# chayanchatterjee/GW-Whisper

Hardware: AMD Instinct MI355X
Metric: 1s-strain segments/sec (encoder fwd) (higher is better)
Workload: dtype bf16; 1 GPU; whisper-tiny encoder fwd, batch 256 log-mel (80x3000) per GPU, 1500 tokens, random-init weights (BASELINE configs[1]); global_batch=256, parallelism=dp1, encoder=tiny, streams_per_gpu=1

## Files before the change

### gw_whisper_amd/csrc/mlp_fused.hip

```cpp
#include "common.h"

#include <stdlib.h>

#include <type_traits>

namespace gww {

namespace {
constexpr int MF_D = 384;
constexpr int MF_KT = MF_D / 64;
constexpr int MF_OT = MF_D / 32;
constexpr int MF_WAVES = 4, MF_THREADS = 256, MF_BM = 128;
#ifndef GWW_MF_EXP
#define GWW_MF_EXP 0
#endif
#ifndef GWW_MF_ABL
#define GWW_MF_ABL 0
#endif
#ifndef GWW_MF_OLDDMA
#define GWW_MF_OLDDMA 0
#endif
#ifndef GWW_MF_AHEAD
#define GWW_MF_AHEAD 3
#endif
#ifndef GWW_MF_SCHED
#define GWW_MF_SCHED 1
#endif
#ifndef GWW_MF_VACC
#define GWW_MF_VACC 1
#endif
#ifndef GWW_MF_NTSTORE
#define GWW_MF_NTSTORE 1
#endif
#ifndef GWW_MF_NTLOAD
#define GWW_MF_NTLOAD 1
#endif
#if GWW_MF_NTLOAD
#define MF_NT " nt"
#else
#define MF_NT ""
#endif
#ifndef GWW_MF_PADNOP
#define GWW_MF_PADNOP 0
#endif
#if GWW_MF_PADNOP
#define MF_PADNOP "s_nop 1\n\t"
#else
#define MF_PADNOP ""
#endif
#ifndef GWW_MF_XLDS
#define GWW_MF_XLDS 0
#endif
#ifndef GWW_MF_XSTNT
#define GWW_MF_XSTNT 0
#endif
#ifndef GWW_MF_XNT
#define GWW_MF_XNT 0
#endif
#if GWW_MF_XNT
#define MF_XNT MF_NT
#else
#define MF_XNT ""
#endif
#ifndef GWW_MF_DMAGAP
#define GWW_MF_DMAGAP 1
#endif
#ifndef GWW_MF_TAIL2
#define GWW_MF_TAIL2 0
#endif
#ifndef GWW_MF_NORM
#define GWW_MF_NORM 1
#endif
#ifndef GWW_MF_XACC
#define GWW_MF_XACC 1
#endif
constexpr int MF_AHEAD = GWW_MF_AHEAD;
constexpr int MF_NST_MAX = MF_AHEAD + 1;
constexpr int MF_TILE = 128 * 64 * 2;
constexpr int MF_GL = 16 / MF_WAVES;
constexpr int MF_FMAX = 1536;
constexpr int MF_SLICE_STRIDE = 144, MF_SLICE_BYTES = 32 * MF_SLICE_STRIDE;
constexpr int MF_OFF_CB = MF_NST_MAX * MF_TILE;
constexpr int MF_OFF_U = MF_OFF_CB + MF_FMAX * 4;
constexpr int MF_OFF_B2 = MF_OFF_U + MF_FMAX * 4;
constexpr int MF_OFF_BO = MF_OFF_B2 + MF_D * 4;
constexpr int MF_OFF_QCB = MF_OFF_BO + MF_D * 4;
constexpr int MF_OFF_SLICE = MF_OFF_QCB + MF_FMAX * 4;
constexpr int MF_LDS = MF_OFF_SLICE + 2 * MF_WAVES * MF_SLICE_BYTES;
static_assert(MF_LDS <= 160 * 1024, "LDS budget");

template <int N>
using MF_FL = std::integral_constant<int, N>;

__device__ __forceinline__ float mf_sum8(float v) {
  v += __builtin_bit_cast(float, __builtin_amdgcn_update_dpp(0, __builtin_bit_cast(int, v), 0xB1, 0xF, 0xF, true));
  v += __builtin_bit_cast(float, __builtin_amdgcn_update_dpp(0, __builtin_bit_cast(int, v), 0x4E, 0xF, 0xF, true));
  v += __builtin_bit_cast(float, __builtin_amdgcn_update_dpp(0, __builtin_bit_cast(int, v), 0x141, 0xF, 0xF, true));
  return v;
}

template <int N>
__device__ __forceinline__ void mf_wait_vmcnt() {
  asm volatile("s_waitcnt vmcnt(%0)" ::"n"(N) : "memory");
}

__device__ __forceinline__ float gelu_sig(float x) {
  const float s = fminf(x * x, 64.0f);
  float q = fmaf(s, 0.0010148164f, -0.1067791331f);
  q = fmaf(s, q, -2.3011178f);
#if GWW_MF_EXP & 32
  const float e = (x * q) * 0.37f;
  return x * ((1.0f + e) * 0.91f);
#else
  const float e = __builtin_amdgcn_exp2f(x * q);
  return x * __builtin_amdgcn_rcpf(1.0f + e);
#endif
}

#ifdef GWW_STAMP
__device__ unsigned long long g_stamp_mlp[24];
#define MSTAMP_DECL unsigned long long _t0 = __builtin_amdgcn_s_memtime(); unsigned long long _acc[20] = {0}; \
  const unsigned long long _tb = _t0, _rb = __builtin_amdgcn_s_memrealtime();
#define MSTAMP(i)                                                  \
  do {                                                             \
    if (GWW_STAMP >= 2 && (i) != 0 && (i) != 3 && (i) != 4 && (i) != 5 && !((i) >= 100)) break; \
    __builtin_amdgcn_sched_barrier(0);                             \
    const unsigned long long _t1 = __builtin_amdgcn_s_memtime();   \
    _acc[(i) >= 100 ? (i) - 100 : (i)] += _t1 - _t0;               \
    _t0 = _t1;                                                     \
    __builtin_amdgcn_sched_barrier(0);                             \
  } while (0)
#define TSTAMP(i) do { if (GWW_STAMP == 3) MSTAMP(100 + (i)); } while (0)
#define MSTAMP_FLUSH                                                                 \
  if (lane == 0) {                                                                   \
    for (int _q = 0; _q < 20; ++_q) atomicAdd(&g_stamp_mlp[_q], _acc[_q]);           \
    atomicAdd(&g_stamp_mlp[21], __builtin_amdgcn_s_memrealtime() - _rb);             \
    atomicAdd(&g_stamp_mlp[22], __builtin_amdgcn_s_memtime() - _tb);                 \
    atomicAdd(&g_stamp_mlp[23], 1ull);                                                \
  }
#else
#define MSTAMP_DECL
#define MSTAMP(i)
#define TSTAMP(i)
#define MSTAMP_FLUSH
#endif
}

__device__ __forceinline__ const float* mf_x0_row(const MfX0& z, const float* X, long g, bool x0, bool& tail, int& seg) {
  tail = false; seg = 0;
  if (!x0) return X + g * MF_D;
  const unsigned b = (unsigned)g / (unsigned)z.T, j = (unsigned)g - b * (unsigned)z.T;
  seg = (int)b;
  tail = (int)j >= z.Tt - 2 && (int)j <= z.T - 2;
  if (tail) return z.pos + (long)j * MF_D;
  return z.xs + ((long)b * z.Tt + ((int)j == z.T - 1 ? z.Tt - 1 : (int)j)) * MF_D;
}

struct MfNoX0 {};
template <int MODE, bool OP, bool X0 = false>
__global__ __launch_bounds__(MF_THREADS, 1) void k_mlp_fused(const float* X, const unsigned short* delta, float* x_out,
                                                            const float* __restrict__ ln_u,
                                                            const float* __restrict__ ln_cb,
                                                            const unsigned short* __restrict__ Wt,
                                                            const float* __restrict__ b2,
                                                            unsigned short* __restrict__ C, long M, int F,
                                                            int stagger_ticks, const float* __restrict__ q_u,
                                                            const float* __restrict__ q_cb,
                                                            unsigned short* __restrict__ q_out, int NQ,
                                                            float* x_next, const float* __restrict__ bo, int keep_x_new,
                                                            const std::conditional_t<X0, MfX0, MfNoX0> z) {
  __shared__ __attribute__((aligned(16))) unsigned char lds[MF_LDS];
  constexpr bool QKV = MODE == 1 || MODE == 2, LNQ = MODE == 2, FIN = MODE == 3;
  static_assert(!X0 || (GWW_MF_NORM && GWW_MF_XACC && (MODE == 2 || (MODE == 1 && OP))), "X0: layer 0's two launches; stages in the u table");
  constexpr bool XACC = GWW_MF_XACC && GWW_MF_NORM && GWW_MF_SCHED && OP && (MODE == 1 || MODE == 3);
  constexpr int MF_NST = MF_AHEAD + 1;
  float* lds_cb = reinterpret_cast<float*>(lds + MF_OFF_CB);
  float* lds_u = reinterpret_cast<float*>(lds + MF_OFF_U);
  float* lds_b2 = reinterpret_cast<float*>(lds + MF_OFF_B2);
  float* lds_bo = reinterpret_cast<float*>(lds + MF_OFF_BO);
  float* lds_qcb = reinterpret_cast<float*>(lds + MF_OFF_QCB);
  constexpr int OP_TILES = OP ? 3 * MF_KT : 0;
  typedef __attribute__((address_space(3))) void* lds_ptr;

  const int tid = threadIdx.x, lane = tid & 63, wave = tid >> 6;
  const int r = lane & 31, hh = lane >> 5;
  const long m_base = (long)blockIdx.x * MF_BM + wave * 32;
  unsigned char* slice = lds + MF_OFF_SLICE + wave * MF_SLICE_BYTES;
  unsigned char* const slice0 = slice;
  const int crow = lane >> 3, cchunk = lane & 7;

  const int wave_u = __builtin_amdgcn_readfirstlane(wave);
  const unsigned lane_off = (unsigned)lane * 16u;
  const unsigned lds_base = (unsigned)(unsigned long long)(lds_ptr)lds;
  auto issue_piece_c = [&](int tile, int stage, auto j_c) {
    constexpr int J = decltype(j_c)::value;
    const unsigned dst = lds_base + (unsigned)(stage * MF_TILE + MF_GL * wave_u * 1024);
    if (GWW_MF_EXP & 8) tile &= 7;
    const unsigned short* src = Wt + ((long)tile * (MF_TILE / 2) + MF_GL * wave_u * 512);
    const unsigned lo = lane_off;
    asm volatile("s_mov_b32 m0, %2\n\ts_nop 0\n\tglobal_load_lds_dwordx4 %0, %1 offset:%3"
                 :
                 : "v"(lo), "s"(src), "s"(dst), "n"(J * 1024)
                 : "memory");
  };
  auto issue_piece = [&](int tile, int stage, int j) {
#if GWW_MF_OLDDMA
    const unsigned dst = lds_base + (unsigned)(stage * MF_TILE + (MF_GL * wave_u + j) * 1024);
    const unsigned short* src = Wt + ((long)tile * (MF_TILE / 2) + (MF_GL * wave_u + j) * 512);
    unsigned keep;
    asm volatile("s_mov_b32 %0, m0\n\ts_mov_b32 m0, %3\n\ts_nop 0\n\tglobal_load_lds_dwordx4 %1, %2\n\ts_mov_b32 m0, %0"
                 : "=&s"(keep) : "v"(lane_off), "s"(src), "s"(dst) : "memory");
#else
    if (j == 0) issue_piece_c(tile, stage, std::integral_constant<int, 0>{});
    else if (j == 1) issue_piece_c(tile, stage, std::integral_constant<int, 1>{});
    else if (j == 2) issue_piece_c(tile, stage, std::integral_constant<int, 2>{});
    else issue_piece_c(tile, stage, std::integral_constant<int, 3>{});
#endif
  };
  auto issue = [&](int tile, int stage) {
#pragma unroll
    for (int j = 0; j < MF_GL; ++j) issue_piece(tile, stage, j);
  };

  MSTAMP_DECL
  auto stage_tables = [&]() {
    for (int i = tid; i < F; i += MF_THREADS) {
      lds_cb[i] = GWW_MF_SCHED ? ln_cb[i] * 0.125f : ln_cb[i];
      if (!GWW_MF_NORM) lds_u[i] = ln_u[i];
    }
    if (!GWW_MF_NORM && FIN) __syncthreads();
    if (!LNQ)
      for (int i = tid; i < MF_D; i += MF_THREADS) lds_b2[i] = XACC ? b2[i] + bo[i] : b2[i];
    if (OP)
      for (int i = tid; i < MF_D; i += MF_THREADS) lds_bo[i] = bo[i];
    if (FIN)
      for (int i = tid; i < MF_D; i += MF_THREADS) { lds_u[i] = q_u[i]; lds_u[MF_D + i] = q_cb[i]; }
    if (QKV && GWW_MF_NORM)
      for (int i = tid; i < NQ; i += MF_THREADS) lds_qcb[i] = q_cb[i];
  };
  if constexpr (!XACC) stage_tables();
  if (stagger_ticks > 0 && blockIdx.x < 256) {
    const unsigned long long t0 = __builtin_amdgcn_s_memrealtime();
    const unsigned long long wait = (unsigned long long)((blockIdx.x >> 3) & 15) * stagger_ticks;
    while (__builtin_amdgcn_s_memrealtime() - t0 < wait) __builtin_amdgcn_s_sleep(8);
  }

#pragma unroll
  for (int p = 0; p < MF_AHEAD; ++p) issue(p, p);
  const long xrow_l = m_base + r < M ? m_base + r : M - 1;
  const unsigned xoff = (unsigned)xrow_l * (unsigned)(MF_D * 4) + 16u * (unsigned)hh;
  f32x4 xp[XACC ? MF_OT : 1][4];
  bool x0 = false;
  int x0_seg0 = 0;
  f32x4* const lds_x0 = reinterpret_cast<f32x4*>(lds + MF_OFF_U);
  const float* x0_stage[2] = {nullptr, nullptr};
  f32x4 x0_sg[2];
  bool x0_tail = false;
  int x0_seg = 0;
  if constexpr (X0) {
    x0 = __builtin_amdgcn_readfirstlane(*z.flag) != 0;
    const unsigned g0 = (unsigned)blockIdx.x * (unsigned)MF_BM;
    x0_seg0 = (int)(g0 / (unsigned)z.T);
    const int seg_last = (int)((unsigned)(M - 1) / (unsigned)z.T);
#pragma unroll
    for (int k = 0; k < 2; ++k) {
      const int q = tid + 256 * k < 4 * (MF_D / 4) ? tid + 256 * k : tid;
      const int sg = q / (2 * (MF_D / 4)), wh = (q / (MF_D / 4)) & 1, c = q % (MF_D / 4);
      const long b = x0_seg0 + sg < seg_last ? x0_seg0 + sg : seg_last;
      x0_stage[k] = (wh ? z.tr + b * MF_D : z.xs + (b * z.Tt + (z.Tt - 2)) * MF_D) + 4 * c;
    }
  }
  auto x0_publish = [&](f32x4 (&sg)[2]) {
    lds_x0[tid] = sg[0];
    if (tid + 256 < 4 * (MF_D / 4)) lds_x0[tid + 256] = sg[1];
    asm volatile("s_waitcnt lgkmcnt(0)" ::: "memory");
    __builtin_amdgcn_s_barrier();
    asm volatile("" ::: "memory");
  };
  if constexpr (XACC && X0) {
    const float* xsrc = mf_x0_row(z, X, xrow_l, x0, x0_tail, x0_seg) + 4 * hh;
#pragma unroll
    for (int t = 0; t < MF_OT; ++t)
#pragma unroll
      for (int cc = 0; cc < 4; ++cc)
        asm volatile("global_load_dwordx4 %0, %1, off offset:%2" MF_XNT : "=a"(xp[t][cc]) : "v"(xsrc), "n"((32 * t + 8 * cc) * 4) : "memory");
#pragma unroll
    for (int k = 0; k < 2; ++k) asm volatile("global_load_dwordx4 %0, %1, off" : "=v"(x0_sg[k]) : "v"(x0_stage[k]) : "memory");
  } else if constexpr (XACC) {
#pragma unroll
    for (int t = 0; t < MF_OT; ++t)
#pragma unroll
      for (int cc = 0; cc < 4; ++cc)
        if (GWW_MF_ABL & 32) asm volatile("v_accvgpr_write_b32 %0, 0" : "=a"(xp[t][cc][0]));
        else asm volatile("global_load_dwordx4 %0, %1, %2 offset:%3" MF_XNT : "=a"(xp[t][cc]) : "v"(xoff), "s"(X), "n"((32 * t + 8 * cc) * 4) : "memory");
  }
  bf16x8 af[MF_KT * 4];
  float row_rstd, row_mean;
  long grow[4];
#pragma unroll
  for (int i = 0; i < 4; ++i) {
    const long g = m_base + 8 * i + crow;
    grow[i] = g < M ? g : M - 1;
  }
  if constexpr (XACC) {
    const unsigned coff = (unsigned)xrow_l * (unsigned)(MF_D * 2) + 64u * (unsigned)hh;
#pragma unroll
    for (int S = 0; S < MF_KT; ++S)
#pragma unroll
      for (int j = 0; j < 4; ++j)
        asm volatile("global_load_dwordx4 %0, %1, %2 offset:%3" : "=v"(af[4 * S + j]) : "v"(coff), "s"(delta), "n"((64 * S + 8 * j) * 2) : "memory");
    if constexpr (X0) {
      if (x0) {
        asm volatile("s_waitcnt vmcnt(24)" : "+v"(x0_sg[0]), "+v"(x0_sg[1]) : : "memory");
#pragma unroll
        for (int t = 0; t < MF_OT; ++t) asm volatile("" : "+a"(xp[t][0]), "+a"(xp[t][1]), "+a"(xp[t][2]), "+a"(xp[t][3]));
        x0_publish(x0_sg);
        if (x0_tail) {
          const f32x4* const st = lds_x0 + (x0_seg - x0_seg0) * (2 * (MF_D / 4)) + hh;
#pragma unroll
          for (int t = 0; t < MF_OT; ++t)
#pragma unroll
            for (int cc = 0; cc < 4; ++cc) {
              const f32x4 xt = st[8 * t + 2 * cc], rt = st[MF_D / 4 + 8 * t + 2 * cc];
#pragma unroll
              for (int k = 0; k < 4; ++k) xp[t][cc][k] = __builtin_fmaf(xt[k], rt[k], xp[t][cc][k]);
            }
        }
      }
    }
    stage_tables();
    asm volatile("s_waitcnt vmcnt(0)" ::: "memory");
#pragma unroll
    for (int i = 0; i < MF_KT * 4; ++i) asm volatile("" : "+v"(af[i]));
    row_rstd = 1.f; row_mean = 0.f;
  } else if constexpr (OP) {
    const unsigned short* crow_p[4];
#pragma unroll
    for (int i = 0; i < 4; ++i) crow_p[i] = delta + grow[i] * MF_D + 8 * cchunk;
    u32x4 cv[MF_KT][4];
#pragma unroll
    for (int S = 0; S < MF_KT; ++S)
#pragma unroll
      for (int i = 0; i < 4; ++i) {
        if (GWW_MF_ABL & 64) { cv[S][i] = u32x4{0x3f803f80u, 0x3f803f80u, 0x3f803f80u, 0x3f803f80u}; continue; }
        asm volatile("global_load_dwordx4 %0, %1, off offset:%2" MF_NT : "=v"(cv[S][i]) : "v"(crow_p[i]), "n"(64 * S * 2) : "memory");
      }
#pragma unroll
    for (int S = 0; S < MF_KT; ++S) {
#pragma unroll
      for (int i = 0; i < 4; ++i) {
        if (!(GWW_MF_ABL & 64)) asm volatile("s_waitcnt vmcnt(%1)" : "+v"(cv[S][i]) : "n"(23 - (4 * S + i)));
        *reinterpret_cast<u32x4*>(slice + (8 * i + crow) * MF_SLICE_STRIDE + cchunk * 16) = cv[S][i];
      }
#pragma unroll
      for (int j = 0; j < 4; ++j) {
        u32x4 u = *reinterpret_cast<const u32x4*>(slice + r * MF_SLICE_STRIDE + (4 * hh + j) * 16);
        asm volatile("" : "+v"(u)::"memory");
        af[4 * S + j] = __builtin_bit_cast(bf16x8, u);
      }
    }
    row_rstd = 1.f; row_mean = 0.f;
  } else
  {
    float s1[4] = {0.f, 0.f, 0.f, 0.f}, s2[4] = {0.f, 0.f, 0.f, 0.f}, cshift[4];
    const float* xrow[4];
    const unsigned short* drow[4];
#pragma unroll
    for (int i = 0; i < 4; ++i) {
      xrow[i] = X + grow[i] * MF_D + 4 * cchunk;
      drow[i] = LNQ ? nullptr : delta + grow[i] * MF_D + 4 * cchunk;
    }
    bool tl[4] = {false, false, false, false};
    const f32x4* st_row[4] = {lds_x0, lds_x0, lds_x0, lds_x0};
    if constexpr (X0) {
#pragma unroll
      for (int i = 0; i < 4; ++i) {
        int seg;
        xrow[i] = mf_x0_row(z, X, grow[i], x0, tl[i], seg) + 4 * cchunk;
        st_row[i] = lds_x0 + (seg - x0_seg0) * (2 * (MF_D / 4)) + cchunk;
      }
#pragma unroll
      for (int k = 0; k < 2; ++k) asm volatile("global_load_dwordx4 %0, %1, off" : "=v"(x0_sg[k]) : "v"(x0_stage[k]) : "memory");
    }
#pragma unroll
    for (int S3 = 0; S3 < MF_KT; S3 += 3) {
      f32x4 xv[3][2][4];
      u32x2 dv[3][2][4];
#pragma unroll
      for (int S = 0; S < 3; ++S)
#pragma unroll
        for (int h2 = 0; h2 < 2; ++h2)
#pragma unroll
          for (int i = 0; i < 4; ++i) {
            if constexpr (X0)
              asm volatile("global_load_dwordx4 %0, %1, off offset:%2"
                           : "=v"(xv[S][h2][i]) : "v"(xrow[i]), "n"((64 * (S3 + S) + 32 * h2) * 4) : "memory");
            else
            asm volatile("global_load_dwordx4 %0, %1, off offset:%2" MF_NT
                         : "=v"(xv[S][h2][i]) : "v"(xrow[i]), "n"((64 * (S3 + S) + 32 * h2) * 4) : "memory");
            if (!LNQ)
              asm volatile("global_load_dwordx2 %0, %1, off offset:%2" MF_NT
                           : "=v"(dv[S][h2][i]) : "v"(drow[i]), "n"((64 * (S3 + S) + 32 * h2) * 2) : "memory");
          }
      if constexpr (X0) {
        if (S3 == 0 && x0) {
          asm volatile("s_waitcnt vmcnt(24)" : "+v"(x0_sg[0]), "+v"(x0_sg[1]) : : "memory");
          x0_publish(x0_sg);
        }
      }
#pragma unroll
      for (int Sl = 0; Sl < 3; ++Sl) {
        const int S = S3 + Sl;
#pragma unroll
        for (int h2 = 0; h2 < 2; ++h2)
#pragma unroll
          for (int i = 0; i < 4; ++i) {
            f32x4 v;
            if (LNQ) {
              asm volatile("s_waitcnt vmcnt(%1)" : "+v"(xv[Sl][h2][i]) : "n"(23 - (8 * Sl + 4 * h2 + i)));
              v = xv[Sl][h2][i];
              if constexpr (X0) {
                if (tl[i]) {
                  const f32x4 xt = st_row[i][16 * S + 8 * h2], rt = st_row[i][MF_D / 4 + 16 * S + 8 * h2];
#pragma unroll
                  for (int k = 0; k < 4; ++k) v[k] = __builtin_fmaf(xt[k], rt[k], v[k]);
                }
              }
            } else {
              asm volatile("s_waitcnt vmcnt(%2)" : "+v"(xv[Sl][h2][i]), "+v"(dv[Sl][h2][i]) : "n"(46 - (8 * Sl + 4 * h2 + i)));
              v = xv[Sl][h2][i];
              v[0] += bf2f((unsigned short)(dv[Sl][h2][i][0] & 0xffff));
              v[1] += bf2f((unsigned short)(dv[Sl][h2][i][0] >> 16));
              v[2] += bf2f((unsigned short)(dv[Sl][h2][i][1] & 0xffff));
              v[3] += bf2f((unsigned short)(dv[Sl][h2][i][1] >> 16));
              *reinterpret_cast<f32x4*>(x_out + grow[i] * MF_D + 64 * S + 32 * h2 + 4 * cchunk) = v;
              asm volatile("" ::: "memory");
            }
            if (S == 0 && h2 == 0) {
              float t = (v[0] + v[1]) + (v[2] + v[3]);
              t = mf_sum8(t);
              cshift[i] = t * (1.0f / 32.0f);
            }
            v[0] -= cshift[i]; v[1] -= cshift[i]; v[2] -= cshift[i]; v[3] -= cshift[i];
            s1[i] += (v[0] + v[1]) + (v[2] + v[3]);
            s2[i] += (v[0] * v[0] + v[1] * v[1]) + (v[2] * v[2] + v[3] * v[3]);
            u32x2 o = {pack2bf(v[0], v[1]), pack2bf(v[2], v[3])};
            *reinterpret_cast<u32x2*>(slice + (8 * i + crow) * MF_SLICE_STRIDE + h2 * 64 + cchunk * 8) = o;
          }
#pragma unroll
        for (int j = 0; j < 4; ++j) {
          u32x4 u = *reinterpret_cast<const u32x4*>(slice + r * MF_SLICE_STRIDE + (4 * hh + j) * 16);
          asm volatile("" : "+v"(u)::"memory");
          af[4 * S + j] = __builtin_bit_cast(bf16x8, u);
        }
      }
    }
    TSTAMP(8);
    float* stat = reinterpret_cast<float*>(slice);
#pragma unroll
    for (int i = 0; i < 4; ++i) {
      float a = s1[i], b = s2[i];
      a = mf_sum8(a); b = mf_sum8(b);
      const float mean = a * (1.0f / MF_D);
      const float var = fmaxf(b * (1.0f / MF_D) - mean * mean, 0.f);
      if (cchunk == 0) {
        stat[8 * i + crow] = rsqrtf(var + 1e-5f);
        stat[32 + 8 * i + crow] = mean;
      }
    }
    row_rstd = stat[r];
    row_mean = stat[32 + r];
    asm volatile("" : "+v"(row_rstd), "+v"(row_mean)::"memory");
    TSTAMP(9);
  }
#if GWW_MF_NORM
  auto normalise_af = [&]() {
    const float nm = -row_mean * row_rstd;
#pragma unroll
    for (int i = 0; i < MF_KT * 4; ++i) {
      u32x4 w = __builtin_bit_cast(u32x4, af[i]);
#pragma unroll
      for (int q = 0; q < 4; ++q)
        w[q] = pack2bf(fmaf(bf2f((unsigned short)(w[q] & 0xffff)), row_rstd, nm), fmaf(bf2f((unsigned short)(w[q] >> 16)), row_rstd, nm));
      af[i] = __builtin_bit_cast(bf16x8, w);
    }
  };
  if (!OP) normalise_af();
#endif
  MSTAMP(0);

  int off1[8], off2[4];
#pragma unroll
  for (int j = 0; j < 8; ++j) off1[j] = r * 256 + ((((j >> 2) * 8 + 4 * hh + (j & 3)) ^ (r & 15)) << 4);
#pragma unroll
  for (int j = 0; j < 4; ++j) off2[j] = r * 128 + (((2 * j + hh) ^ ((r >> 1) & 7)) << 4);
  int offq[4];
#pragma unroll
  for (int j = 0; j < 4; ++j) offq[j] = r * 128 + (((4 * hh + j) ^ ((r >> 1) & 7)) << 4);

  f32x16 sacc[4], oacc[MF_OT];
  if constexpr (XACC) {
#pragma unroll
    for (int t = 0; t < MF_OT; ++t) {
      asm volatile("" : "+a"(xp[t][0]), "+a"(xp[t][1]), "+a"(xp[t][2]), "+a"(xp[t][3]));
      const auto lo = __builtin_shufflevector(xp[t][0], xp[t][1], 0, 1, 2, 3, 4, 5, 6, 7);
      const auto hi = __builtin_shufflevector(xp[t][2], xp[t][3], 0, 1, 2, 3, 4, 5, 6, 7);
      oacc[t] = __builtin_shufflevector(lo, hi, 0, 1, 2, 3, 4, 5, 6, 7, 8, 9, 10, 11, 12, 13, 14, 15);
    }
  } else {
#pragma unroll
    for (int t = 0; t < MF_OT; ++t)
#pragma unroll
      for (int j = 0; j < 16; ++j) oacc[t][j] = 0.f;
  }
  u32x4 pf[4][2];

  float a_u[2][4], a_b[2][4], a_v[2][4];
  auto act_begin = [&](int slot, int c, int p) {
    if (GWW_MF_EXP & 2) return;
    if (GWW_MF_SCHED) {
      a_b[slot][0] = a_b[slot][1] = a_b[slot][2] = a_b[slot][3] = 0.f;
      return;
    }
    const int nl = 128 * c + 32 * (p >> 2) + 8 * (p & 3) + 4 * hh;
#if !GWW_MF_NORM
    const float4 uv = *reinterpret_cast<const float4*>(lds_u + nl);
    a_u[slot][0] = uv.x; a_u[slot][1] = uv.y; a_u[slot][2] = uv.z; a_u[slot][3] = uv.w;
#endif
    if (GWW_MF_EXP & 16) {
      a_b[slot][0] = a_b[slot][1] = a_b[slot][2] = a_b[slot][3] = row_rstd;
      return;
    }
    const float4 bv = *reinterpret_cast<const float4*>(lds_cb + nl);
    a_b[slot][0] = bv.x; a_b[slot][1] = bv.y; a_b[slot][2] = bv.z; a_b[slot][3] = bv.w;
  };
  auto act_val = [&](int slot, int p, int e) {
    if (GWW_MF_EXP & 2) {
      a_v[slot][e] = sacc[p >> 2][4 * (p & 3) + e];
      return;
    }
#if GWW_MF_SCHED
    a_v[slot][e] = 0.125f * gelu_sig(8.0f * sacc[p >> 2][4 * (p & 3) + e]);
#elif GWW_MF_NORM
    a_v[slot][e] = gelu_sig(sacc[p >> 2][4 * (p & 3) + e] + a_b[slot][e]);
#else
    a_v[slot][e] = gelu_sig(fmaf(row_rstd, fmaf(-row_mean, a_u[slot][e], sacc[p >> 2][4 * (p & 3) + e]), a_b[slot][e]));
#endif
  };
  auto act_end = [&](int slot, int p) {
    const int t = p >> 2, cc = p & 3;
    pf[t][cc >> 1][2 * (cc & 1)] = pack2bf(a_v[slot][0], a_v[slot][1]);
    pf[t][cc >> 1][2 * (cc & 1) + 1] = pack2bf(a_v[slot][2], a_v[slot][3]);
    asm volatile("" : "+v"(pf[t][cc >> 1][2 * (cc & 1)]), "+v"(pf[t][cc >> 1][2 * (cc & 1) + 1]));
  };
  auto act_piece = [&](int slot, int c, int p) {
    act_begin(slot, c, p);
    act_val(slot, p, 0); act_val(slot, p, 1); act_val(slot, p, 2); act_val(slot, p, 3);
    act_end(slot, p);
  };

  float g_t[4] = {0.f, 0.f, 0.f, 0.f}, g_w[4] = {0.f, 0.f, 0.f, 0.f}, g_q[4] = {0.f, 0.f, 0.f, 0.f};
#define MF_FENCE()                                                                                                       \
  asm volatile("" : "+v"(g_t[0]), "+v"(g_t[1]), "+v"(g_t[2]), "+v"(g_t[3]), "+v"(g_w[0]), "+v"(g_w[1]), "+v"(g_w[2]),   \
               "+v"(g_w[3]), "+v"(g_q[0]), "+v"(g_q[1]), "+v"(g_q[2]), "+v"(g_q[3]))
  auto preload_bias = [&](int t, int chunk, int q) {
    const float4 bv = *reinterpret_cast<const float4*>(lds_cb + 64 * chunk + 32 * (t & 1) + 8 * q + 4 * hh);
    sacc[t][4 * q] = bv.x; sacc[t][4 * q + 1] = bv.y; sacc[t][4 * q + 2] = bv.z; sacc[t][4 * q + 3] = bv.w;
  };
  auto gelu_slice = [&](int t, int g) {
    if (GWW_MF_EXP & 2) return;
    const int k = g / 12, j = g % 12;
#pragma unroll
    for (int pr = 0; pr < 2; ++pr) {
      const int op = j - pr;
      if (op < 0 || op > 8) continue;
#pragma unroll
      for (int sl = 0; sl < 2; ++sl) {
        const int i = 2 * pr + sl, v = 4 * k + i;
        const float S_ = sacc[t][v];
        float& T_ = g_t[i];
        float& W_ = g_w[i];
        float& Q_ = g_q[i];
        if (op == 0) asm("v_mul_f32_e64 %0, %1, %1 clamp" : "=v"(W_) : "v"(S_));
        else if (op == 1) Q_ = fmaf(W_, 33.2535038f, -54.67091615f);
        else if (op == 2) Q_ = fmaf(W_, Q_, -18.4089424f);
        else if (op == 3) W_ = S_ * Q_;
        else if (op == 4) W_ = __builtin_amdgcn_exp2f(W_);
        else if (op == 5) W_ = 1.0f + W_;
        else if (op == 6) W_ = __builtin_amdgcn_rcpf(W_);
        else if (op == 7) T_ = S_ * W_;
        else if (op == 8 && sl == 1) {
          pf[t][k >> 1][2 * (k & 1) + pr] = pack2bf(g_t[2 * pr], g_t[2 * pr + 1]);
          asm volatile("" : "+v"(pf[t][k >> 1][2 * (k & 1) + pr]));
        }
      }
    }
  };

// ... 586 lines not shown
      const float4 bv = *reinterpret_cast<const float4*>(lds_qcb + 64 * chunk + 32 * (t & 1) + 8 * q + 4 * hh);
      sacc[t][4 * q] = bv.x; sacc[t][4 * q + 1] = bv.y; sacc[t][4 * q + 2] = bv.z; sacc[t][4 * q + 3] = bv.w;
    };
    auto q_ride = [&](auto q_c, auto g_c, int chunk, auto mode_c) {
      constexpr int Q = decltype(q_c)::value, G = decltype(g_c)::value, RM = decltype(mode_c)::value;
      if constexpr (RM == 1 && G >= 4 && G < 12) {
        constexpr int tt = (G - 4) >> 2, cc = (G - 4) & 3;
        const f32x16& a = sacc[2 * Q + tt];
        u32x2 o = {pack2bf(a[4 * cc], a[4 * cc + 1]), pack2bf(a[4 * cc + 2], a[4 * cc + 3])};
        *reinterpret_cast<u32x2*>(slice + r * MF_SLICE_STRIDE + (32 * tt + 8 * cc + 4 * hh) * 2) = o;
      }
      if constexpr (RM >= 1 && G >= 12 && G < 20) {
        if (chunk + 1 < nchunks) q_preload(2 * Q + ((G - 12) >> 2), chunk + 1, (G - 12) & 3);
      }
      if constexpr (RM == 1 && G >= 22 && G < 26) {
        tq[G - 22] = *reinterpret_cast<const u32x4*>(slice + (8 * (G - 22) + crow) * MF_SLICE_STRIDE + cchunk * 16);
        asm volatile("" : "+v"(tq[G - 22]));
      }
      if constexpr (RM == 1 && G >= 37 && G < 41) {
        const long orow = m_base + 8 * (G - 37) + crow;
        if (!(GWW_MF_ABL & 1))
          __builtin_nontemporal_store(tq[G - 37], reinterpret_cast<u32x4*>(q_out + orow * NQ + (chunk - 1) * 64 + 8 * cchunk));
      }
    };
    auto run_qtile = [&](auto flat_c, auto par_c, auto idx3_c, auto mode_c, int chunk, auto extra_c, auto nowait_c) {
      constexpr int FLAT = decltype(flat_c)::value, PAR = decltype(par_c)::value, IDX3 = decltype(idx3_c)::value;
      constexpr int RM = decltype(mode_c)::value, EXTRA = decltype(extra_c)::value;
      constexpr bool NOWAIT = decltype(nowait_c)::value != 0;
      constexpr int ST = (12 % MF_NST == 0) ? ((FLAT + OP_TILES) % MF_NST) : -1;
      if (ST >= 0) stage = ST;
      if (!(GWW_MF_ABL & 4)) {
        if (!NOWAIT) mf_wait_vmcnt<MF_GL*(MF_AHEAD - 2) + ((GWW_MF_ABL & 3) ? 0 : EXTRA)>();
      }
      if (!(GWW_MF_ABL & 8)) __builtin_amdgcn_s_barrier();
      TSTAMP(6);
      const int dma_tile = it + MF_AHEAD < total ? it + MF_AHEAD : total - 1;
      const int dma_stage = stage + MF_AHEAD >= MF_NST ? stage + MF_AHEAD - MF_NST : stage + MF_AHEAD;
      const int stage_next = stage + 1 == MF_NST ? 0 : stage + 1;
#pragma unroll
      for (int sub = 0; sub < 4; ++sub) {
        bf16x8(&cur)[4] = wf[sub & 1];
        bf16x8(&nxt)[4] = wf[(sub + 1) & 1];
        const unsigned char* Wn = lds + (sub == 3 ? stage_next : stage) * MF_TILE;
        __builtin_amdgcn_sched_barrier(0);
#pragma unroll
        for (int u = 0; u < 4; ++u) {
          const int tl = u & 1, ks = 2 * sub + (u >> 1);
          asm volatile("s_nop 1\n\tv_mfma_f32_32x32x16_bf16 %0, %1, %2, %0" : "+v"(sacc[2 * PAR + tl]) : "v"(cur[u]), "v"(af[8 * IDX3 + ks]));
          if (u < 3) asm volatile("" : "+v"(cur[u + 1]));
          else if (sub < 3) asm volatile("" : "+v"(nxt[0]));
          {
            const int off = sub == 3 ? first_off(0, u) : (u & 1) * 8192 + off1[2 * (sub + 1) + (u >> 1)];
            nxt[u] = *reinterpret_cast<const bf16x8*>(Wn + off);
          }
          if constexpr (RM != 0) {
            if (sub == 0 && u == 0) q_ride(MF_FL<1 - PAR>{}, MF_FL<16 * IDX3 + 0>{}, chunk, mode_c);
            else if (sub == 0 && u == 1) q_ride(MF_FL<1 - PAR>{}, MF_FL<16 * IDX3 + 1>{}, chunk, mode_c);
            else if (sub == 0 && u == 2) q_ride(MF_FL<1 - PAR>{}, MF_FL<16 * IDX3 + 2>{}, chunk, mode_c);
            else if (sub == 0 && u == 3) q_ride(MF_FL<1 - PAR>{}, MF_FL<16 * IDX3 + 3>{}, chunk, mode_c);
            else if (sub == 1 && u == 0) q_ride(MF_FL<1 - PAR>{}, MF_FL<16 * IDX3 + 4>{}, chunk, mode_c);
            else if (sub == 1 && u == 1) q_ride(MF_FL<1 - PAR>{}, MF_FL<16 * IDX3 + 5>{}, chunk, mode_c);
            else if (sub == 1 && u == 2) q_ride(MF_FL<1 - PAR>{}, MF_FL<16 * IDX3 + 6>{}, chunk, mode_c);
            else if (sub == 1 && u == 3) q_ride(MF_FL<1 - PAR>{}, MF_FL<16 * IDX3 + 7>{}, chunk, mode_c);
            else if (sub == 2 && u == 0) q_ride(MF_FL<1 - PAR>{}, MF_FL<16 * IDX3 + 8>{}, chunk, mode_c);
            else if (sub == 2 && u == 1) q_ride(MF_FL<1 - PAR>{}, MF_FL<16 * IDX3 + 9>{}, chunk, mode_c);
            else if (sub == 2 && u == 2) q_ride(MF_FL<1 - PAR>{}, MF_FL<16 * IDX3 + 10>{}, chunk, mode_c);
            else if (sub == 2 && u == 3) q_ride(MF_FL<1 - PAR>{}, MF_FL<16 * IDX3 + 11>{}, chunk, mode_c);
            else if (sub == 3 && u == 0) q_ride(MF_FL<1 - PAR>{}, MF_FL<16 * IDX3 + 12>{}, chunk, mode_c);
            else if (sub == 3 && u == 1) q_ride(MF_FL<1 - PAR>{}, MF_FL<16 * IDX3 + 13>{}, chunk, mode_c);
            else if (sub == 3 && u == 2) q_ride(MF_FL<1 - PAR>{}, MF_FL<16 * IDX3 + 14>{}, chunk, mode_c);
            else q_ride(MF_FL<1 - PAR>{}, MF_FL<16 * IDX3 + 15>{}, chunk, mode_c);
          }
          if (!(GWW_MF_ABL & 4)) {
            const int piece = 4 * sub + u - (9 - 4 * IDX3);
            if (piece >= 0 && piece < 4) issue_piece(dma_tile, dma_stage, piece);
          }
        }
        __builtin_amdgcn_sched_barrier(0);
      }
      stage = stage_next;
      ++it;
      TSTAMP(7);
    };
    using NW = std::conditional_t<LNQ || (GWW_MF_ABL & 32), I0, I1>;
    if (LNQ) {
#pragma unroll
      for (int u = 0; u < 4; ++u) wf[0][u] = *reinterpret_cast<const bf16x8*>(lds + stage * MF_TILE + first_off(0, u));
    }
#pragma unroll
    for (int t = 0; t < 2; ++t)
#pragma unroll
      for (int q = 0; q < 4; ++q) q_preload(t, 0, q);
    run_qtile(MF_FL<0>{}, I0{}, I0{}, I2{}, 0, I0{}, NW{});
    run_qtile(MF_FL<1>{}, I0{}, I1{}, I2{}, 0, I0{}, NW{});
    run_qtile(MF_FL<2>{}, I0{}, I2{}, I2{}, 0, I0{}, I0{});
    run_qtile(MF_FL<3>{}, I1{}, I0{}, I1{}, 1, I0{}, I0{});
    run_qtile(MF_FL<4>{}, I1{}, I1{}, I1{}, 1, I0{}, I0{});
    run_qtile(MF_FL<5>{}, I1{}, I2{}, I1{}, 1, I0{}, I0{});
    using I4 = std::integral_constant<int, 4>;
    for (int c = 2; c < nchunks; c += 4) {
      run_qtile(MF_FL<6>{}, I0{}, I0{}, I1{}, c, I4{}, I0{});
      run_qtile(MF_FL<7>{}, I0{}, I1{}, I1{}, c, I4{}, I0{});
      run_qtile(MF_FL<8>{}, I0{}, I2{}, I1{}, c, I0{}, I0{});
      run_qtile(MF_FL<9>{}, I1{}, I0{}, I1{}, c + 1, I4{}, I0{});
      run_qtile(MF_FL<10>{}, I1{}, I1{}, I1{}, c + 1, I4{}, I0{});
      run_qtile(MF_FL<11>{}, I1{}, I2{}, I1{}, c + 1, I0{}, I0{});
      run_qtile(MF_FL<12>{}, I0{}, I0{}, I1{}, c + 2, I4{}, I0{});
      run_qtile(MF_FL<13>{}, I0{}, I1{}, I1{}, c + 2, I4{}, I0{});
      run_qtile(MF_FL<14>{}, I0{}, I2{}, I1{}, c + 2, I0{}, I0{});
      run_qtile(MF_FL<15>{}, I1{}, I0{}, I1{}, c + 3, I4{}, I0{});
      run_qtile(MF_FL<16>{}, I1{}, I1{}, I1{}, c + 3, I4{}, I0{});
      run_qtile(MF_FL<17>{}, I1{}, I2{}, I1{}, c + 3, I0{}, I0{});
    }
    asm volatile("s_nop 15\n\ts_nop 15" : "+v"(sacc[2]), "+v"(sacc[3]));
    if (!(GWW_MF_ABL & 2)) {
#pragma unroll
      for (int tt = 0; tt < 2; ++tt)
#pragma unroll
        for (int cc = 0; cc < 4; ++cc) {
          const f32x16& a = sacc[2 + tt];
          u32x2 o = {pack2bf(a[4 * cc], a[4 * cc + 1]), pack2bf(a[4 * cc + 2], a[4 * cc + 3])};
          *reinterpret_cast<u32x2*>(slice + r * MF_SLICE_STRIDE + (32 * tt + 8 * cc + 4 * hh) * 2) = o;
        }
#pragma unroll
      for (int i = 0; i < 4; ++i) {
        const u32x4 u = *reinterpret_cast<const u32x4*>(slice + (8 * i + crow) * MF_SLICE_STRIDE + cchunk * 16);
        const long orow = m_base + 8 * i + crow;
        if (GWW_MF_ABL & 1) { asm volatile("" :: "v"(u)); continue; }
        __builtin_nontemporal_store(u, reinterpret_cast<u32x4*>(q_out + orow * NQ + (nchunks - 1) * 64 + 8 * cchunk));
      }
    }
    mf_wait_vmcnt<(GWW_MF_ABL & 3) ? 0 : 8>();
    }
#else
    const int T0 = OP_TILES + 6 * nck;
    if (LNQ) {
#pragma unroll
      for (int u = 0; u < 4; ++u) wf[0][u] = *reinterpret_cast<const bf16x8*>(lds + stage * MF_TILE + u * 4096 + offq[0]);
    }
    f32x16 acc[4];
    for (int nt = 0; nt < NQ / 128; ++nt) {
#if GWW_MF_SCHED
#pragma unroll
      for (int t = 0; t < 4; ++t)
#pragma unroll
        for (int cc = 0; cc < 4; ++cc) {
          const float4 bv = *reinterpret_cast<const float4*>(lds_qcb + 128 * nt + 32 * t + 8 * cc + 4 * hh);
          acc[t][4 * cc] = bv.x; acc[t][4 * cc + 1] = bv.y; acc[t][4 * cc + 2] = bv.z; acc[t][4 * cc + 3] = bv.w;
        }
#endif
#pragma unroll
      for (int kt = 0; kt < MF_KT; ++kt) {
        constexpr int TAIL_ST = (GWW_MF_ABL & 3) ? 0 : 8;
        if (GWW_MF_ABL & 4) {}
        else if (XACC && nt == 0 && kt <= MF_AHEAD - 2) mf_wait_vmcnt<MF_GL*(MF_AHEAD - 2) + ((GWW_MF_ABL & 16) ? 0 : 4 * MF_OT)>();
        else if (!LNQ && !(GWW_MF_ABL & 32) && nt == 0 && kt <= MF_AHEAD - 2) {}
        else if (nt > 0 && kt <= MF_AHEAD - 2) mf_wait_vmcnt<MF_GL*(MF_AHEAD - 2) + TAIL_ST>();
        else mf_wait_vmcnt<MF_GL*(MF_AHEAD - 2)>();
        if (!(GWW_MF_ABL & 8)) __builtin_amdgcn_s_barrier();
        TSTAMP(6);
        const int itq = T0 + nt * MF_KT + kt;
        const int dma_tile = itq + MF_AHEAD < total ? itq + MF_AHEAD : total - 1;
        const int dma_stage = stage + MF_AHEAD >= MF_NST ? stage + MF_AHEAD - MF_NST : stage + MF_AHEAD;
        const int stage_next = stage + 1 == MF_NST ? 0 : stage + 1;
#pragma unroll
        for (int sub = 0; sub < 4; ++sub) {
          const int q = 4 * kt + sub;
          bf16x8(&cur)[4] = wf[q & 1];
          bf16x8(&nxt)[4] = wf[(q + 1) & 1];
          const unsigned char* Wn = lds + (sub == 3 ? stage_next : stage) * MF_TILE + offq[(sub + 1) & 3];
          __builtin_amdgcn_sched_barrier(0);
          if (!(GWW_MF_ABL & 4)) issue_piece(dma_tile, dma_stage, sub);
#pragma unroll
          for (int u = 0; u < 4; ++u) {
#if GWW_MF_SCHED
            asm volatile(MF_PADNOP "v_mfma_f32_32x32x16_bf16 %0, %1, %2, %0" : "+v"(acc[u]) : "v"(cur[u]), "v"(af[4 * kt + sub]));
#else
            if (kt == 0 && sub == 0) {
              f32x16 z;
#pragma unroll
              for (int j = 0; j < 16; ++j) z[j] = 0.f;
              acc[u] = __builtin_amdgcn_mfma_f32_32x32x16_bf16(cur[u], af[4 * kt + sub], z, 0, 0, 0);
            } else {
              acc[u] = __builtin_amdgcn_mfma_f32_32x32x16_bf16(cur[u], af[4 * kt + sub], acc[u], 0, 0, 0);
            }
#endif
            nxt[u] = *reinterpret_cast<const bf16x8*>(Wn + u * 4096);
          }
#if !GWW_MF_SCHED
          __builtin_amdgcn_sched_group_barrier(0x008, 1, 0);
          __builtin_amdgcn_sched_group_barrier(0x100, 1, 0);
          __builtin_amdgcn_sched_group_barrier(0x002, 2, 0);
          __builtin_amdgcn_sched_group_barrier(0x008, 1, 0);
          __builtin_amdgcn_sched_group_barrier(0x100, 1, 0);
          __builtin_amdgcn_sched_group_barrier(0x002, 2, 0);
          __builtin_amdgcn_sched_group_barrier(0x008, 1, 0);
          __builtin_amdgcn_sched_group_barrier(0x100, 1, 0);
          __builtin_amdgcn_sched_group_barrier(0x002, 2, 0);
          __builtin_amdgcn_sched_group_barrier(0x008, 1, 0);
          __builtin_amdgcn_sched_group_barrier(0x100, 1, 0);
          __builtin_amdgcn_sched_group_barrier(0x002, 2, 0);
#endif
          __builtin_amdgcn_sched_barrier(0);
        }
        stage = stage_next;
        TSTAMP(7);
      }
#if GWW_MF_SCHED
      asm volatile("s_nop 15\n\ts_nop 15" : "+v"(acc[0]), "+v"(acc[1]), "+v"(acc[2]), "+v"(acc[3]));
#endif
#pragma unroll
      for (int half = 0; half < 2; ++half) {
        if (GWW_MF_ABL & 2) break;
#pragma unroll
        for (int tt = 0; tt < 2; ++tt) {
          const int t = 2 * half + tt;
#pragma unroll
          for (int cc = 0; cc < 4; ++cc) {
            const int nl = 128 * nt + 32 * t + 8 * cc + 4 * hh;
#if GWW_MF_SCHED
            const float v0 = acc[t][4 * cc], v1 = acc[t][4 * cc + 1], v2 = acc[t][4 * cc + 2], v3 = acc[t][4 * cc + 3];
            (void)nl;
#elif GWW_MF_NORM
            const float4 bv = *reinterpret_cast<const float4*>(lds_qcb + nl);
            const float v0 = acc[t][4 * cc] + bv.x, v1 = acc[t][4 * cc + 1] + bv.y;
            const float v2 = acc[t][4 * cc + 2] + bv.z, v3 = acc[t][4 * cc + 3] + bv.w;
#else
            const float4 bv = *reinterpret_cast<const float4*>(lds_qcb + nl);
            const float4 uv = *reinterpret_cast<const float4*>(lds_u + nl);
            const float v0 = fmaf(row_rstd, fmaf(-row_mean, uv.x, acc[t][4 * cc]), bv.x);
            const float v1 = fmaf(row_rstd, fmaf(-row_mean, uv.y, acc[t][4 * cc + 1]), bv.y);
            const float v2 = fmaf(row_rstd, fmaf(-row_mean, uv.z, acc[t][4 * cc + 2]), bv.z);
            const float v3 = fmaf(row_rstd, fmaf(-row_mean, uv.w, acc[t][4 * cc + 3]), bv.w);
#endif
            u32x2 o = {pack2bf(v0, v1), pack2bf(v2, v3)};
            *reinterpret_cast<u32x2*>(slice + r * MF_SLICE_STRIDE + (32 * tt + 8 * cc + 4 * hh) * 2) = o;
          }
        }
#pragma unroll
        for (int i = 0; i < 4; ++i) {
          const u32x4 u = *reinterpret_cast<const u32x4*>(slice + (8 * i + crow) * MF_SLICE_STRIDE + cchunk * 16);
          const long orow = m_base + 8 * i + crow;
          if (GWW_MF_ABL & 1) { asm volatile("" :: "v"(u)); continue; }
#if GWW_MF_NTSTORE
          __builtin_nontemporal_store(u, reinterpret_cast<u32x4*>(q_out + orow * NQ + nt * 128 + 64 * half + 8 * cchunk));
#else
          *reinterpret_cast<u32x4*>(q_out + orow * NQ + nt * 128 + 64 * half + 8 * cchunk) = u;
#endif
        }
      }
    }
    mf_wait_vmcnt<(GWW_MF_ABL & 3) ? 0 : 8>();
#endif
  }
  MSTAMP(3);
  MSTAMP_FLUSH
}

__device__ __forceinline__ u32x4 mf_scale_bf16x8(u32x4 v, float f) {
#pragma unroll
  for (int j = 0; j < 4; ++j) {
    const float lo = __uint_as_float(v[j] << 16) * f, hi = __uint_as_float(v[j] & 0xffff0000u) * f;
    v[j] = (__float_as_uint(lo) >> 16) | (__float_as_uint(hi) & 0xffff0000u);
  }
  return v;
}

__global__ __launch_bounds__(256) void k_mlp_pack(const unsigned short* __restrict__ w1,
                                                  const unsigned short* __restrict__ w2,
                                                  const unsigned short* __restrict__ wq,
                                                  unsigned short* __restrict__ out, int F, long n_chunks16,
                                                  const unsigned short* __restrict__ wo) {
  const int nck = F / 64, mlp_tiles = 6 * nck, op_tiles = wo ? 3 * MF_KT : 0;
  for (long g = (long)blockIdx.x * 256 + threadIdx.x; g < n_chunks16; g += (long)gridDim.x * 256) {
    const int tile_all = (int)(g >> 10), within = (int)(g & 1023);
    const int row = within >> 3, chunk = (within & 7) ^ ((row >> 1) & 7);
    const int tile = tile_all - op_tiles;
    u32x4 v;
    if (tile < 0) {
      const int nt = tile_all / MF_KT, kt = tile_all - nt * MF_KT;
      v = *reinterpret_cast<const u32x4*>(wo + (long)(128 * nt + row) * MF_D + 64 * kt + 8 * chunk);
    } else if (tile >= mlp_tiles) {
#if GWW_MF_TAIL2
      const int it2 = tile - mlp_tiles, cq = it2 / 3, k3 = it2 - 3 * cq;
      const int row2 = within >> 4, ch = (within & 15) ^ (row2 & 15);
      v = *reinterpret_cast<const u32x4*>(wq + (long)(64 * cq + row2) * MF_D + 128 * k3 + 8 * ch);
#else
      const int it2 = tile - mlp_tiles, nt = it2 / MF_KT, kt = it2 - nt * MF_KT;
      v = *reinterpret_cast<const u32x4*>(wq + (long)(128 * nt + row) * MF_D + 64 * kt + 8 * chunk);
#endif
    } else {
      int kind, cp, idx3;
      if (tile < 3) { kind = 0; cp = 0; idx3 = tile; }
      else {
        const int k = tile - 3, blk = k / 6, w = k - 6 * blk;
        if (blk == nck - 1) { kind = 1; cp = blk; idx3 = w; }
        else if (w < 3) { kind = 0; cp = blk + 1; idx3 = w; }
        else { kind = 1; cp = blk; idx3 = w - 3; }
      }
      if (kind == 0) {
        const int row2 = within >> 4, ch = (within & 15) ^ (row2 & 15);
        v = *reinterpret_cast<const u32x4*>(w1 + (long)(64 * cp + row2) * MF_D + 128 * idx3 + 8 * ch);
        if (GWW_MF_SCHED) v = mf_scale_bf16x8(v, 0.125f);
      } else {
        const unsigned short* src = w2 + (long)(128 * idx3 + row) * F + 64 * cp;
        unsigned short e[8];
#pragma unroll
        for (int j = 0; j < 8; ++j) {
          const int p = 8 * chunk + j;
          e[j] = src[(p & ~12) | ((p & 4) << 1) | ((p & 8) >> 1)];
        }
        v = u32x4{(unsigned)e[0] | ((unsigned)e[1] << 16), (unsigned)e[2] | ((unsigned)e[3] << 16),
                  (unsigned)e[4] | ((unsigned)e[5] << 16), (unsigned)e[6] | ((unsigned)e[7] << 16)};
        if (GWW_MF_SCHED) v = mf_scale_bf16x8(v, 8.0f);
      }
    }
    reinterpret_cast<u32x4*>(out)[g] = v;
  }
}

int launch_mlp_pack(const void* w1_folded, const void* w2, const void* wqkv_folded, void* out, int d, int F, int NQ,
                    hipStream_t s, const void* wo) {
  GWW_REQUIRE(d == MF_D && F % 128 == 0 && F >= 0 && (F > 0 || wqkv_folded),
              "mlp_pack: d must be 384 and ffn a multiple of 128 (0: only the q / k / v panel, for LayerNorm 1 + q / k / v alone)");
  GWW_REQUIRE(!wqkv_folded || (NQ > 0 && NQ % 128 == 0), "mlp_pack: the q / k / v panel needs NQ %% 128 == 0");
// ... 162 lines not shown
```

Measured before the change: 26650 segments/s.

## Shrink LDS layout for LNQ mode to fit two workgroups per CU

Introduces a per-mode LDS layout template. MODE 2 (LN+QKV) uses a 3-stage pipeline and a smaller table set so that two workgroups fit per CU, with launch bounds raised accordingly. The MODE 2 loop also switches to issuing a whole tile's DMA at sub 0 rather than one piece per sub-step, computes the stage index statically from kt, and tweaks the variance accumulation. The aim is to hide latency through higher occupancy. The cost is a shallower prefetch depth and register pressure capped by the 2-WG launch bound.

```diff
diff --git a/gw_whisper_amd/csrc/mlp_fused.hip b/gw_whisper_amd/csrc/mlp_fused.hip
--- a/gw_whisper_amd/csrc/mlp_fused.hip
+++ b/gw_whisper_amd/csrc/mlp_fused.hip
@@ -74,20 +74,35 @@
 #ifndef GWW_MF_XACC
 #define GWW_MF_XACC 1
 #endif
-constexpr int MF_AHEAD = GWW_MF_AHEAD;
-constexpr int MF_NST_MAX = MF_AHEAD + 1;
 constexpr int MF_TILE = 128 * 64 * 2;
 constexpr int MF_GL = 16 / MF_WAVES;
 constexpr int MF_FMAX = 1536;
 constexpr int MF_SLICE_STRIDE = 144, MF_SLICE_BYTES = 32 * MF_SLICE_STRIDE;
-constexpr int MF_OFF_CB = MF_NST_MAX * MF_TILE;
-constexpr int MF_OFF_U = MF_OFF_CB + MF_FMAX * 4;
-constexpr int MF_OFF_B2 = MF_OFF_U + MF_FMAX * 4;
-constexpr int MF_OFF_BO = MF_OFF_B2 + MF_D * 4;
-constexpr int MF_OFF_QCB = MF_OFF_BO + MF_D * 4;
-constexpr int MF_OFF_SLICE = MF_OFF_QCB + MF_FMAX * 4;
-constexpr int MF_LDS = MF_OFF_SLICE + 2 * MF_WAVES * MF_SLICE_BYTES;
-static_assert(MF_LDS <= 160 * 1024, "LDS budget");
+template <int MODE>
+struct MfLay {
+  static constexpr int AHEAD = GWW_MF_AHEAD;
+  static constexpr int NST = AHEAD + 1;
+  static constexpr int WG_PER_CU = 1;
+  static constexpr int OFF_CB = NST * MF_TILE;
+  static constexpr int OFF_U = OFF_CB + MF_FMAX * 4;
+  static constexpr int OFF_B2 = OFF_U + MF_FMAX * 4;
+  static constexpr int OFF_BO = OFF_B2 + MF_D * 4;
+  static constexpr int OFF_QCB = OFF_BO + MF_D * 4;
+  static constexpr int OFF_SLICE = OFF_QCB + MF_FMAX * 4;
+  static constexpr int LDS = OFF_SLICE + 2 * MF_WAVES * MF_SLICE_BYTES;
+  static_assert(LDS <= 160 * 1024, "LDS budget");
+};
+template <>
+struct MfLay<2> {
+  static constexpr int AHEAD = 2, NST = AHEAD + 1;
+  static constexpr int WG_PER_CU = 2;
+  static constexpr int OFF_QCB = NST * MF_TILE;
+  static constexpr int OFF_U = OFF_QCB + MF_FMAX * 4;
+  static constexpr int OFF_SLICE = OFF_U + 4 * MF_D * 4;
+  static constexpr int OFF_CB = OFF_QCB, OFF_B2 = OFF_QCB, OFF_BO = OFF_QCB;
+  static constexpr int LDS = OFF_SLICE + MF_WAVES * MF_SLICE_BYTES;
+  static_assert(LDS <= 80 * 1024, "two workgroups per CU: half of the 160 KB");
+};
 
 template <int N>
 using MF_FL = std::integral_constant<int, N>;
@@ -158,7 +173,7 @@
 
 struct MfNoX0 {};
 template <int MODE, bool OP, bool X0 = false>
-__global__ __launch_bounds__(MF_THREADS, 1) void k_mlp_fused(const float* X, const unsigned short* delta, float* x_out,
+__global__ __launch_bounds__(MF_THREADS, MfLay<MODE>::WG_PER_CU) void k_mlp_fused(const float* X, const unsigned short* delta, float* x_out,
                                                             const float* __restrict__ ln_u,
                                                             const float* __restrict__ ln_cb,
                                                             const unsigned short* __restrict__ Wt,
@@ -169,23 +184,24 @@
                                                             unsigned short* __restrict__ q_out, int NQ,
                                                             float* x_next, const float* __restrict__ bo, int keep_x_new,
                                                             const std::conditional_t<X0, MfX0, MfNoX0> z) {
-  __shared__ __attribute__((aligned(16))) unsigned char lds[MF_LDS];
+  using LAY = MfLay<MODE>;
+  __shared__ __attribute__((aligned(16))) unsigned char lds[LAY::LDS];
   constexpr bool QKV = MODE == 1 || MODE == 2, LNQ = MODE == 2, FIN = MODE == 3;
   static_assert(!X0 || (GWW_MF_NORM && GWW_MF_XACC && (MODE == 2 || (MODE == 1 && OP))), "X0: layer 0's two launches; stages in the u table");
   constexpr bool XACC = GWW_MF_XACC && GWW_MF_NORM && GWW_MF_SCHED && OP && (MODE == 1 || MODE == 3);
-  constexpr int MF_NST = MF_AHEAD + 1;
-  float* lds_cb = reinterpret_cast<float*>(lds + MF_OFF_CB);
-  float* lds_u = reinterpret_cast<float*>(lds + MF_OFF_U);
-  float* lds_b2 = reinterpret_cast<float*>(lds + MF_OFF_B2);
-  float* lds_bo = reinterpret_cast<float*>(lds + MF_OFF_BO);
-  float* lds_qcb = reinterpret_cast<float*>(lds + MF_OFF_QCB);
+  constexpr int MF_AHEAD = LAY::AHEAD, MF_NST = LAY::NST;
+  float* lds_cb = reinterpret_cast<float*>(lds + LAY::OFF_CB);
+  float* lds_u = reinterpret_cast<float*>(lds + LAY::OFF_U);
+  float* lds_b2 = reinterpret_cast<float*>(lds + LAY::OFF_B2);
+  float* lds_bo = reinterpret_cast<float*>(lds + LAY::OFF_BO);
+  float* lds_qcb = reinterpret_cast<float*>(lds + LAY::OFF_QCB);
   constexpr int OP_TILES = OP ? 3 * MF_KT : 0;
   typedef __attribute__((address_space(3))) void* lds_ptr;
 
   const int tid = threadIdx.x, lane = tid & 63, wave = tid >> 6;
   const int r = lane & 31, hh = lane >> 5;
   const long m_base = (long)blockIdx.x * MF_BM + wave * 32;
-  unsigned char* slice = lds + MF_OFF_SLICE + wave * MF_SLICE_BYTES;
+  unsigned char* slice = lds + LAY::OFF_SLICE + wave * MF_SLICE_BYTES;
   unsigned char* const slice0 = slice;
   const int crow = lane >> 3, cchunk = lane & 7;
 
@@ -224,7 +240,7 @@
 
   MSTAMP_DECL
   auto stage_tables = [&]() {
-    for (int i = tid; i < F; i += MF_THREADS) {
+    for (int i = tid; i < (LNQ ? 0 : F); i += MF_THREADS) {
       lds_cb[i] = GWW_MF_SCHED ? ln_cb[i] * 0.125f : ln_cb[i];
       if (!GWW_MF_NORM) lds_u[i] = ln_u[i];
     }
@@ -252,7 +268,7 @@
   f32x4 xp[XACC ? MF_OT : 1][4];
   bool x0 = false;
   int x0_seg0 = 0;
-  f32x4* const lds_x0 = reinterpret_cast<f32x4*>(lds + MF_OFF_U);
+  f32x4* const lds_x0 = reinterpret_cast<f32x4*>(lds + LAY::OFF_U);
   const float* x0_stage[2] = {nullptr, nullptr};
   f32x4 x0_sg[2];
   bool x0_tail = false;
@@ -442,8 +458,17 @@
               cshift[i] = t * (1.0f / 32.0f);
             }
             v[0] -= cshift[i]; v[1] -= cshift[i]; v[2] -= cshift[i]; v[3] -= cshift[i];
-            s1[i] += (v[0] + v[1]) + (v[2] + v[3]);
-            s2[i] += (v[0] * v[0] + v[1] * v[1]) + (v[2] * v[2] + v[3] * v[3]);
+            if constexpr (LNQ) {
+              float p0 = v[0] * v[0], p1 = v[1] * v[1], p2 = v[2] * v[2], p3 = v[3] * v[3];
+              asm volatile("" : "+v"(p0), "+v"(p1), "+v"(p2), "+v"(p3));
+              const float q23 = (S == 0 && h2 == 0) ? __builtin_fmaf(v[2], v[2], p3) : p2 + p3;
+              s1[i] += (v[0] + v[1]) + (v[2] + v[3]);
+              s2[i] += (p0 + p1) + q23;
+              asm volatile("" : "+v"(s1[i]), "+v"(s2[i]));
+            } else {
+              s1[i] += (v[0] + v[1]) + (v[2] + v[3]);
+              s2[i] += (v[0] * v[0] + v[1] * v[1]) + (v[2] * v[2] + v[3] * v[3]);
+            }
             u32x2 o = {pack2bf(v[0], v[1]), pack2bf(v[2], v[3])};
             *reinterpret_cast<u32x2*>(slice + (8 * i + crow) * MF_SLICE_STRIDE + h2 * 64 + cchunk * 8) = o;
           }
@@ -1336,6 +1361,7 @@
 #pragma unroll
       for (int kt = 0; kt < MF_KT; ++kt) {
         constexpr int TAIL_ST = (GWW_MF_ABL & 3) ? 0 : 8;
+        if constexpr (LNQ) stage = kt % MF_NST;
         if (GWW_MF_ABL & 4) {}
         else if (XACC && nt == 0 && kt <= MF_AHEAD - 2) mf_wait_vmcnt<MF_GL*(MF_AHEAD - 2) + ((GWW_MF_ABL & 16) ? 0 : 4 * MF_OT)>();
         else if (!LNQ && !(GWW_MF_ABL & 32) && nt == 0 && kt <= MF_AHEAD - 2) {}
@@ -1354,7 +1380,9 @@
           bf16x8(&nxt)[4] = wf[(q + 1) & 1];
           const unsigned char* Wn = lds + (sub == 3 ? stage_next : stage) * MF_TILE + offq[(sub + 1) & 3];
           __builtin_amdgcn_sched_barrier(0);
-          if (!(GWW_MF_ABL & 4)) issue_piece(dma_tile, dma_stage, sub);
+          if (GWW_MF_ABL & 4) {}
+          else if (LNQ) { if (sub == 0) issue(dma_tile, dma_stage); }
+          else issue_piece(dma_tile, dma_stage, sub);
 #pragma unroll
           for (int u = 0; u < 4; ++u) {
 #if GWW_MF_SCHED
```

After: 26850 segments/s (median of 6 runs). About the same (+0.8%).
